# BoothGroup/evcont

Measured on AMD Instinct MI355X. Metric: continuation geometries/sec (energy+force), H30 STO-3G, 20 training states, higher is better.
Workload: dtype f64

## Files before the change

### evcont_amd/csrc/kernels.hpp

```cpp
#pragma once
#include "common.hpp"

namespace evc {

constexpr int kMaxOrbitals = 96;
constexpr int kMaxBatchG = 32;

struct RowProblem {
    const double *A;
    const double *v;
    double *partial;
    int64_t rows, cols, ld, vstride, pstride;
    int nspans, nblocks;
    int64_t span_cols;
    int lds_plan;
};
struct GemvRowsLaunch {
    RowProblem p[2];
    int nblk0;
    int nblk1;
    int tpg[2], trem[2], nrg[2];
};
struct ColProblem {
    const double *A;
    const double *w;
    const double *wt;
    double *out;
    int64_t rows, cols, ld, wstride, ostride;
    double *part;
    int64_t pstride;
};
constexpr int kColSlabs = 64;
struct GemvColsLaunch {
    ColProblem p[2];
    int nblk0;
};
int launch_gemv_rows_mfma(const GemvRowsLaunch &L, int g0, int G, int tiles, hipStream_t st);
int launch_gemv_cols_mfma(GemvColsLaunch L, int g0, int G, hipStream_t st);
void plan_rows(RowProblem &P, bool batched);
bool rows_lds_applicable(const RowProblem &p0, const RowProblem &p1);
void plan_rows_lds(RowProblem &p0, RowProblem &p1);
int rows_max_spans(const RowProblem &P, bool small);
int launch_gemv_rows_lds(const GemvRowsLaunch &L, int g0, int G, hipStream_t st);
int rows_lds_max_g(const RowProblem &p0, const RowProblem &p1);
int cols_lds_mode(const ColProblem &p0, const ColProblem &p1, int G);
int launch_gemv_cols_lds(const GemvColsLaunch &L, int g0, int G, hipStream_t st);
int launch_gemv_cols_lds_slab(const GemvColsLaunch &L, int g0, int G, hipStream_t st);
bool rows_groups_all_mfma(int count);
size_t rows_ws_doubles(int64_t rows, int64_t cols);
int launch_gemv_rows(RowProblem p0, RowProblem p1, int count, hipStream_t st);
int launch_gemv_cols(ColProblem p0, ColProblem p1, int count, hipStream_t st);

int launch_quarter_transform(const double *in, int64_t sin, const double *C, int64_t sC, int c_transposed, int n,
                             double *out, int64_t sout, int count, hipStream_t st);
struct PairTransformArgs {
    const double *in;
    const double *C;
    double *out;
    double *packed;
    double *k3;
    int64_t sin, sC, sout, spacked, sk3, packed_len;
    double diag_mult;
    int ct, n;
    int tiles_per_wg;
    int sym8;
    int lead_sym;
    int in_lower;
    int rs_lower;
    int out_pairs;
    int in_pairs;
    int in_ld, out_ld;
};
__host__ __device__ inline int pair_ld(int n) { return (n * (n + 1) / 2 + 15) & ~15; }
constexpr int kPairTransformMaxN = 32;
constexpr int kPtRawMax = (kPairTransformMaxN * (kPairTransformMaxN + 1) / 2 + 1 + 127) / 128;
constexpr int kPtRowLen = kPtRawMax * 128 + 4;
int launch_pair_transform(const PairTransformArgs &a, int count, hipStream_t st);
bool pair_transform_dma_applicable(const PairTransformArgs &a, int count);
int launch_pair_transform_dma(const PairTransformArgs &a, int count, hipStream_t st);
bool y2_dma_applicable(int n);
int launch_y2_dma(const double *SB, const double *M1, const double *X, int64_t sX, int n, double *partial, int64_t sws,
                  int count, int slabs, int tiles_per_wg, int ppt, hipStream_t st);
int launch_pack(const double *h2, int64_t sh2, int n, double diag_mult, double *out, int64_t sout, int64_t out_len,
                int count, hipStream_t st);
int launch_pack_sym8(const double *h2, int64_t sh2, int n, double diag_mult, double *out, int64_t sout,
                     int64_t out_len, int count, hipStream_t st);
int launch_unpack(const double *packed, int64_t sp, int n, double *out, int64_t sout, int count, hipStream_t st);
int launch_sym_oao_t(const double *G, int64_t sG, int n, double *out, int64_t sout, int count, hipStream_t st);
int launch_unpack_sym(const double *packed, int64_t sp, int n, double *GsT, double *SB, int64_t sws, double *G,
                      int64_t sG, int count, hipStream_t st);
int launch_unpack8(const double *packed, int64_t sp, int n, double *SB, int64_t sws, double *G, int64_t sG, int count,
                   int lead_half, hipStream_t st);
int launch_y2_sb(const double *SB, const double *K3, int n, double *partial, int64_t sws, int count, hipStream_t st);
int launch_y2_fused(const double *SB, const double *M1, const double *X, int64_t sX, int n, double *partial,
                    int64_t sws, int count, hipStream_t st);
int y2_fused_slabs(int n, int count);
bool y2_fused_available(int n);
int y2_slabs(int n);
int y2_slab_capacity(int n);
int launch_y2(const double *GsT, const double *K3, int n, double *partial, int64_t sws, int count, hipStream_t st);
int ip1_chunks(int n);
__host__ __device__ inline int64_t geo_of(int64_t g, int geo_period) { return geo_period > 0 ? g % geo_period : g; }
struct Ip1Args {
    const double *ip1;
    const double *Gao;
    double *t2part;
    const double *dh;
    const double *Pao;
    double *term3;
    const double *y2part;
    double *y2;
    int64_t sip1, sdh, sws;
    int n, natm, nslab, nchunk;
    int presym;
    int fold_cd;
    int ip1_s2kl;
    int geo_period;
    int slots;
};
constexpr int kIp1MaxSlots = 8;
int launch_ip1_dh(const Ip1Args &a, int count, hipStream_t st);

bool pair64_applicable(const PairTransformArgs &a);
int launch_pair_transform64(const PairTransformArgs &a, int count, hipStream_t st);
bool y2_64_applicable(int n);
int y2_64_slabs(int n, int count);
int launch_y2_64(const double *SB, const double *M1, const double *X, int64_t sX, int n, double *partial, int64_t sws,
                 int count, hipStream_t st);

struct LoewdinArgs {
    const double *S, *h;
    double *X, *U, *s, *h1;
    int64_t sS, sh, sws;
    int n;
    int warm;
    int fast;
    double *scratch;
    int64_t sscratch;
    double *flag;
    int part;
};
int launch_loewdin(const LoewdinArgs &a, int count, hipStream_t st);
bool loewdin_split_available(int n);
int launch_loewdin_big(const LoewdinArgs &a, int count, hipStream_t st);
int eigh_fast_enabled();
int subspace_few_enabled();

struct SolveArgs {
    const double *h1part;
    int nsp1;
    double alpha1;
    const double *h2part;
    int nsp2;
    double alpha2;
    const double *S;
    int64_t sS;
    int T, layout, nroots;
    double e_shift;
    const double *e_shift_dev;
    double *evals, *evecs, *Hout;
    double *w2, *w1;
    double *w2t;
    double *w1t;
    int64_t sh1, sh2, sev, svec, sH, sw;
    int64_t w2_offset, w2_count;
    double *vstd;
    int warm;
    int fast;
    double *bcache;
    int few;
    double *scratch;
    int64_t sscratch;
};
constexpr int kSubspaceSmallT = 32;
constexpr int kSubspaceMaxT = 512;
int launch_subspace_loewdin(const SolveArgs &s, const LoewdinArgs &l, int count, hipStream_t st);
int launch_subspace_solve(const SolveArgs &a, int count, hipStream_t st);
size_t subspace_big_scratch_doubles(int T);
int launch_subspace_big(const SolveArgs &a, int count, hipStream_t st);

__host__ __device__ inline bool layout_pairs(int layout) {
    return layout == EVC_LAYOUT_PAIR5 || layout == EVC_LAYOUT_PACK2 || layout == EVC_LAYOUT_SYM8;
}
int launch_pair_weights(const double *c, int T, int layout, double *w1, double *w2, int64_t w2_offset,
                        int64_t w2_count, hipStream_t st);
int launch_pair_weights_geo(const double *c, int64_t sc, int geo_period, int T, int layout, const int32_t *pairs,
                            int npairs, double *w1, double *w2, double *w1t, double *w2t, int64_t sw, int64_t w2_offset,
                            int64_t w2_count, hipStream_t st);
constexpr int kPairWeightsSlots = 256;
struct PairWeightsArgs {
    const double *c;
    double *w1, *w2;
    double *w1t, *w2t;
    int64_t sw, w2_offset, w2_count, sc;
    int T, pairs, slot0, geo_period;
    int16_t k[kPairWeightsSlots], l[kPairWeightsSlots];
};
struct GradPrepArgs {
    int n;
    const double *X;
    const double *hcore;
    const double *D;
    double *Pao;
    double *Y1;
    int64_t sws, sh, sD;
    double scale1;
    int geo_period;
};
int launch_grad_prep(const GradPrepArgs &a, int count, hipStream_t st);
int launch_unpack8_prep(const GradPrepArgs &a, const double *packed, int64_t sp, double *SB, int64_t sws, int count,
                        hipStream_t st);
struct GradFinalArgs {
    int n, natm;
    const double *U, *s;
    const double *Y1;
    const double *y2;
    const double *ipovlp;
    const int64_t *aoslices;
    const double *t2part;
    int nchunk;
    const double *term3;
    const double *gnuc;
    double scale1;
    double *grad;
    int64_t sws, sip, sgn, sgrad;
    int geo_period;
};
int launch_grad_final(const GradFinalArgs &a, int count, hipStream_t st);

}
```

### evcont_amd/csrc/pair_dma.hip

```cpp
#include <stdlib.h>

#include "common.hpp"
#include "kernels.hpp"

namespace evc {

namespace {

typedef double d4 __attribute__((ext_vector_type(4)));
typedef double d2 __attribute__((ext_vector_type(2)));

constexpr int kPdMaxN = 30;
constexpr unsigned kPdRaw = 4;
constexpr unsigned kPdRB = kPdRaw * 1024 + 64;
constexpr unsigned kPdStage = 4 * kPdRB;
constexpr unsigned kPdP = 3872;
constexpr unsigned kPdTab = kPdStage + 16 * kPdP;
constexpr unsigned kPdLds = kPdTab, kPdLds1 = kPdTab + 512 * 4;

__device__ __forceinline__ d4 mfma_f64(double a, double b, d4 c) {
    return __builtin_amdgcn_mfma_f64_16x16x4f64(a, b, c, 0, 0, 0);
}
__device__ __forceinline__ void glds16(unsigned voff, const void *sbase, unsigned lds_addr) {
    asm volatile("s_mov_b32 m0, %2\n\ts_nop 0\n\tglobal_load_lds_dwordx4 %0, %1"
                 :
                 : "v"(voff), "s"(sbase), "s"(lds_addr)
                 : "memory");
}
__device__ __forceinline__ void gstore16(unsigned voff, d2 v, const void *sbase) {
    asm volatile("global_store_dwordx4 %0, %1, %2" : : "v"(voff), "v"(v), "s"(sbase) : "memory");
}
__device__ __forceinline__ unsigned opaque(unsigned x) {
    asm volatile("" : "+v"(x));
    return x;
}
typedef __attribute__((address_space(3))) double lds_f64;
typedef __attribute__((address_space(3))) float lds_f32;
typedef float f2 __attribute__((ext_vector_type(2)));
typedef __attribute__((address_space(3))) f2 lds_f2;
__device__ __forceinline__ double lds_ld(unsigned addr) { return *(lds_f64 *)(uintptr_t)addr; }
__device__ __forceinline__ void lds_st(unsigned addr, double v) { *(lds_f64 *)(uintptr_t)addr = v; }
__device__ __forceinline__ void wait_vm_dyn(int k) {
    if (k <= 0) asm volatile("s_waitcnt vmcnt(0)" ::: "memory");
    else if (k == 1) asm volatile("s_waitcnt vmcnt(1)" ::: "memory");
    else if (k == 2) asm volatile("s_waitcnt vmcnt(2)" ::: "memory");
    else asm volatile("s_waitcnt vmcnt(3)" ::: "memory");
}

#ifdef EVC_PTD_NO_SETPRIO
#define EVC_PTD_PRIO(x_) do { } while (0)
#else
#define EVC_PTD_PRIO(x_) __builtin_amdgcn_s_setprio(x_)
#endif

}

template <int MODE>
__global__ __launch_bounds__(256, 2) void ptd_kernel(PairTransformArgs a) {
    constexpr int KS = 8, NT = 2;
    extern __shared__ __align__(16) char lds[];
    const int n = a.n;
    const int npairs = n * (n + 1) / 2;
    const int in_ld = a.in_ld ? a.in_ld : npairs, out_ld = a.out_ld;
    const int64_t g = blockIdx.y;
    const double *__restrict__ in = a.in + g * a.sin;
    const double *__restrict__ C = a.C + g * a.sC;
    const int ntiles = (npairs + 7) / 8;
    const int t_begin = blockIdx.x * a.tiles_per_wg, t_end = min(ntiles, t_begin + a.tiles_per_wg);
    if (t_begin >= t_end) return;
    const int niter = 2 * (t_end - t_begin);
    const int lane = threadIdx.x & 63;
    const int wave = __builtin_amdgcn_readfirstlane(threadIdx.x >> 6);
    const int l15 = lane & 15, l4 = lane >> 4;

    const int e0 = 8 * t_begin + wave;
    const int dw = (int)(((reinterpret_cast<uintptr_t>(in) >> 3) + (uintptr_t)((int64_t)e0 * in_ld)) & 1);
    const unsigned rowb = (unsigned)wave * kPdRB;
    unsigned fa[NT][KS];
#pragma unroll
    for (int rt = 0; rt < NT; ++rt)
#pragma unroll
        for (int kk = 0; kk < KS; ++kk) {
            const int r = rt * 16 + l15, s = 4 * kk + l4;
            const int hi = s > r ? s : r, lo = s > r ? r : s;
            fa[rt][kk] = (r < n && s < n) ? rowb + 8u * (unsigned)(dw + hi * (hi + 1) / 2 + lo) : rowb + kPdRaw * 1024;
        }
    if (lane < 8) *reinterpret_cast<double *>(lds + rowb + kPdRaw * 1024 + 8 * lane) = 0.0;
    const unsigned wbytes = (unsigned)(((npairs + dw) * 8 + 15) & ~15);
    unsigned vo[kPdRaw];
#pragma unroll
    for (unsigned u = 0; u < kPdRaw; ++u) {
        const unsigned o = 1024u * u + 16u * (unsigned)lane;
        vo[u] = o < wbytes ? o : 0u;
    }
    const int npieces = __builtin_amdgcn_readfirstlane((int)((wbytes + 1023u) >> 10));
    auto dma_row = [&](int e) {
        const int ec = e < npairs ? e : wave;
        const char *src = reinterpret_cast<const char *>(in + (int64_t)ec * in_ld) - 8 * dw;
#pragma unroll
        for (unsigned u = 0; u < kPdRaw; ++u)
            if ((int)u < npieces) glds16(vo[u], src, rowb + 1024u * u);
    };
    dma_row(e0);

    double xf[KS][NT];
#pragma unroll
    for (int kk = 0; kk < KS; ++kk)
#pragma unroll
        for (int t = 0; t < NT; ++t) {
            const int d = 4 * kk + l4, c = t * 16 + l15;
            const bool ok = d < n && c < n;
            const double *src = C + (ok ? (a.ct ? c * n + d : d * n + c) : 0);
            const double v = *src;
            xf[kk][t] = ok ? v : 0.0;
        }

    unsigned sa[2][12];
#pragma unroll
    for (int f = 0; f < 12; ++f) {
        const int tile = f / 4, reg = f % 4;
        const int it = tile == 0 ? 0 : 1, st = tile == 2 ? 1 : 0;
        const int r2 = it * 16 + l4 + 4 * reg, s2 = st * 16 + l15;
        const bool ok = r2 < n && s2 <= r2;
        sa[0][f] = opaque(kPdStage + (unsigned)wave * kPdP + 8u * (unsigned)(ok ? r2 * (r2 + 1) / 2 + s2 : npairs + l15));
        sa[1][f] = opaque(sa[0][f] + 8u * kPdP);
    }
    const int wl = 2 * (threadIdx.x & 3), ur = threadIdx.x >> 2;
    const unsigned wo = opaque(kPdStage + (unsigned)wl * kPdP + 8u * (unsigned)ur);
    const unsigned gvo = (unsigned)((ur * out_ld + wl) * 8);
    char *outg = reinterpret_cast<char *>(MODE == 0 ? a.out + g * a.sout : a.packed + g * a.spacked);
    [[maybe_unused]] unsigned tv[8];
    [[maybe_unused]] double frow[8];
    if constexpr (MODE == 1) {
        for (int u = threadIdx.x; u < 512; u += 256) {
            const int r = tri_row_small(u);
            *(lds_f32 *)(uintptr_t)(kPdTab + 4u * (unsigned)u) = (u == r * (r + 3) / 2) ? 1.0f : 2.0f;
        }
        if (blockIdx.x == 0) {
            double *pk = a.packed + g * a.spacked;
            const int64_t M = (int64_t)npairs * (npairs + 1) / 2;
            for (int64_t m = M + threadIdx.x; m < a.packed_len; m += 256) pk[m] = 0.0;
        }
        __syncthreads();
#pragma unroll
        for (int k = 0; k < 8; ++k) {
            const int u = ur + 64 * k;
            tv[k] = (unsigned)((u * (u + 1) / 2 + wl) * 8);
            frow[k] = (double)*(lds_f32 *)(uintptr_t)(kPdTab + 4u * (unsigned)(u & 511));
        }
    }
    const int wrows = npairs - 16 * wave;
    int vmask = 0;
#pragma unroll
    for (int k = 0; k < 8; ++k) vmask |= (64 * k < wrows) ? 1 << k : 0;
    vmask = __builtin_amdgcn_readfirstlane(vmask);
    int cntA = 0, cntB = 0;
#pragma unroll
    for (int c = 1; c < 4; ++c) {
        cntA += (64 * c < wrows) ? 1 : 0;
        cntB += (64 * (4 + c) < wrows) ? 1 : 0;
    }

    double mf[NT][KS];
    asm volatile("s_waitcnt vmcnt(0)" ::: "memory");
#pragma unroll
    for (int rt = 0; rt < NT; ++rt)
#pragma unroll
        for (int kk = 0; kk < KS; ++kk) mf[rt][kk] = lds_ld(fa[rt][kk]);
    asm volatile("s_waitcnt lgkmcnt(0)" ::: "memory");
    dma_row(e0 + 4);

    d4 nnA[NT][NT], nnB[NT][NT];
#pragma unroll
    for (int it = 0; it < NT; ++it)
#pragma unroll
        for (int st = 0; st < NT; ++st) nnA[it][st] = nnB[it][st] = (d4){0.0, 0.0, 0.0, 0.0};
    const d4 zero = {0.0, 0.0, 0.0, 0.0};

    auto iteration = [&](auto compute_tag, auto ph_tag, const int i, d4 (&nnp)[NT][NT], d4 (&nn)[NT][NT]) {
        constexpr bool COMPUTE = decltype(compute_tag)::value;
        constexpr int PH = decltype(ph_tag)::value;
        constexpr bool ODD = (PH & 1) != 0;
        constexpr unsigned TP = PH >> 1;
        d4 h[NT][NT];
        if constexpr (COMPUTE || !ODD) {
            constexpr unsigned simm = ODD ? 0u : 4u * kPdP, sbuf = ODD ? TP : (TP ^ 1u);
#pragma unroll
            for (int kk = 0; kk < KS; ++kk) {
#pragma unroll
                for (int m = 0; m < NT * NT; ++m) {
                    if constexpr (COMPUTE) {
                        const int rt = m / NT, st = m % NT;
                        EVC_PTD_PRIO(0);
                        h[rt][st] = mfma_f64(mf[rt][kk], xf[kk][st], kk == 0 ? zero : h[rt][st]);
                        EVC_PTD_PRIO(1);
                    }
                    const int f = kk * 2 + m;
                    if (m < 2 && f < 12) {
                        const int tile = f / 4, reg = f % 4;
                        const int it = tile == 0 ? 0 : 1, st2 = tile == 2 ? 1 : 0;
                        lds_st(sa[sbuf][f] + simm, nnp[it][st2][reg]);
                    }
                    __builtin_amdgcn_sched_barrier(0);
                }
            }
        }
        if (!ODD && i >= 2) lds_barrier();
        {
            int act = (ODD ? i >= 3 : i >= 2) ? vmask : 0;
            const int jt = (ODD ? i - 3 : i - 2) >> 1;
            constexpr unsigned bimm = (TP ^ 1u) * 8u * kPdP;
            char *ob = outg + (int64_t)(8 * (t_begin + jt)) * 8;
#ifdef EVC_PTD_K0
            const int K = 0;
#else
            const int K = (MODE == 0 && i >= 3) ? (ODD ? cntA : cntB) : 0;
#endif
            d2 dv[4];
            [[maybe_unused]] int kd = 0;
            [[maybe_unused]] d2 cf = {1.0, 1.0};
            if constexpr (MODE == 1) {
                const int tg = t_begin + (jt < 0 ? 0 : jt);
                kd = tg >> 3;
                act &= ~((1 << kd) - 1);
                ob = outg + (int64_t)(8 * tg) * 8;
                const f2 c2 = *(lds_f2 *)(uintptr_t)(kPdTab + 4u * (unsigned)(8 * tg + wl));
                cf = (d2){(double)c2[0], (double)c2[1]};
            }
            asm volatile("" : "+s"(act));
#pragma unroll
            for (int kk = 0; kk < KS; ++kk) {
                if ((kk & 1) == 0) {
                    const int c = kk / 2, k = (ODD ? 4 : 0) + c;
                    if (act >> k & 1) {
                        dv[c][0] = lds_ld(wo + 512u * k + bimm);
                        dv[c][1] = lds_ld(wo + 512u * k + bimm + kPdP);
                    }
                }
                __builtin_amdgcn_sched_barrier(0);
#pragma unroll
                for (int m = 0; m < 3; ++m) {
                    if constexpr (COMPUTE) {
                        const int it = m == 0 ? 0 : 1, st = m == 2 ? 1 : 0;
                        EVC_PTD_PRIO(0);
                        nn[it][st] = mfma_f64(xf[kk][it], h[kk / 4][st][kk % 4], kk == 0 ? zero : nn[it][st]);
                        EVC_PTD_PRIO(1);
                        if (m == 0) {
                            if (kk == 0) wait_vm_dyn(K);
                            if (kk < 2) {
#pragma unroll
                                for (int k2 = 0; k2 < KS; ++k2)
                                    mf[kk][k2] = lds_ld(fa[kk][k2]);
                            }
                            if (kk == 2) {
                                asm volatile("s_waitcnt lgkmcnt(0)" ::: "memory");
                                dma_row(e0 + 4 * (i + 2));
                            }
                        }
                    }
                    if (m == 2 && (kk & 1) == 1) {
                        const int c = kk / 2, k = (ODD ? 4 : 0) + c;
                        if constexpr (MODE == 0) {
                            if (act >> k & 1) gstore16(gvo, dv[c], ob + (int64_t)(64 * k) * out_ld * 8);
                        } else if (act >> k & 1) {
                            const int u = ur + 64 * k;
                            d2 f = cf * frow[k];
                            if (k != kd) {
                                const d2 v = dv[c] * f;
                                if (u < npairs) gstore16(tv[k], v, ob);
                            } else {
                                const int d = u - (8 * (t_begin + jt) + wl);
                                if (d == 0) f[0] *= a.diag_mult;
                                if (d == 1) f[1] *= a.diag_mult;
                                const d2 v = dv[c] * f;
                                if (u < npairs) {
                                    if (d >= 1) *reinterpret_cast<d2 *>(ob + tv[k]) = v;
                                    else if (d == 0) *reinterpret_cast<double *>(ob + tv[k]) = v[0];
                                }
                            }
                        }
                    }
                    __builtin_amdgcn_sched_barrier(0);
                }
            }
        }
    };
    using T = std::true_type;
    using F = std::false_type;
    using P0 = std::integral_constant<int, 0>;
    using P1 = std::integral_constant<int, 1>;
    using P2 = std::integral_constant<int, 2>;
    using P3 = std::integral_constant<int, 3>;
    int i = 0;
    for (; i + 4 <= niter; i += 4) {
        iteration(T{}, P0{}, i, nnB, nnA);
        iteration(T{}, P1{}, i + 1, nnA, nnB);
        iteration(T{}, P2{}, i + 2, nnB, nnA);
        iteration(T{}, P3{}, i + 3, nnA, nnB);
    }
    if (i < niter) {
        iteration(T{}, P0{}, i, nnB, nnA);
        iteration(T{}, P1{}, i + 1, nnA, nnB);
        iteration(F{}, P2{}, i + 2, nnB, nnA);
        iteration(F{}, P3{}, i + 3, nnA, nnB);
    } else {
        iteration(F{}, P0{}, i, nnB, nnA);
        iteration(F{}, P1{}, i + 1, nnA, nnB);
    }
    asm volatile("s_waitcnt vmcnt(0)" ::: "memory");
}

__global__ __launch_bounds__(256, 2) void y2d_kernel(const double *__restrict__ SB, const double *__restrict__ M1,
                                                     const double *__restrict__ X, int64_t sX, int n,
                                                     double *__restrict__ partial, int64_t sws, int tiles_per_wg, int ppt) {
    constexpr int KS = 8, NT = 2, NPAD = 32;
    extern __shared__ __align__(16) char lds[];
    const int npairs = n * (n + 1) / 2, ld = pair_ld(n);
    const int64_t g = blockIdx.y;
    SB += g * sws;
    M1 += g * sws;
    X += g * sX;
    partial += g * sws;
    const int ntiles = (npairs + ppt - 1) / ppt;
    const int t_begin = blockIdx.x * tiles_per_wg, t_end = min(ntiles, t_begin + tiles_per_wg);
    const int lane = threadIdx.x & 63;
    const int wave = __builtin_amdgcn_readfirstlane(threadIdx.x >> 6);
    const int l15 = lane & 15, l4 = lane >> 4;
    d4 yD[NT][NT], yO[NT][NT];
#pragma unroll
    for (int ti = 0; ti < NT; ++ti)
#pragma unroll
        for (int ta = 0; ta < NT; ++ta) yD[ti][ta] = yO[ti][ta] = (d4){0.0, 0.0, 0.0, 0.0};
    if (t_begin < t_end) {
        const int niter = (ppt / 4) * (t_end - t_begin);
        const unsigned rowM = (unsigned)wave * 2u * kPdRB, rowT = rowM + kPdRB;
        unsigned fa[NT][KS];
#pragma unroll
        for (int rt = 0; rt < NT; ++rt)
#pragma unroll
            for (int kk = 0; kk < KS; ++kk) {
                const int r = rt * 16 + l15, s = 4 * kk + l4;
                const int hi = s > r ? s : r, lo = s > r ? r : s;
                fa[rt][kk] = opaque((r < n && s < n) ? rowM + 8u * (unsigned)(hi * (hi + 1) / 2 + lo) : rowM + kPdRaw * 1024);
            }
        if (lane < 8) {
            *reinterpret_cast<double *>(lds + rowM + kPdRaw * 1024 + 8 * lane) = 0.0;
            *reinterpret_cast<double *>(lds + rowT + kPdRaw * 1024 + 8 * lane) = 0.0;
        }
        const unsigned wbytes = (unsigned)((npairs * 8 + 15) & ~15);
        unsigned vo[kPdRaw];
#pragma unroll
        for (unsigned u = 0; u < kPdRaw; ++u) {
            const unsigned o = 1024u * u + 16u * (unsigned)lane;
            vo[u] = o < wbytes ? o : 0u;
        }
        const int npieces = __builtin_amdgcn_readfirstlane((int)((wbytes + 1023u) >> 10));
        auto dma_row = [&](const double *base, int e, unsigned dst) {
            const char *src = reinterpret_cast<const char *>(base + (int64_t)(e < npairs ? e : wave) * ld);
#pragma unroll
            for (unsigned u = 0; u < kPdRaw; ++u)
                if ((int)u < npieces) glds16(vo[u], src, dst + 1024u * u);
        };
        auto wait_older = [&]() {
            if (npieces >= 4) asm volatile("s_waitcnt vmcnt(4)" ::: "memory");
            else if (npieces == 3) asm volatile("s_waitcnt vmcnt(3)" ::: "memory");
            else if (npieces == 2) asm volatile("s_waitcnt vmcnt(2)" ::: "memory");
            else asm volatile("s_waitcnt vmcnt(1)" ::: "memory");
        };
        const int e0 = ppt * t_begin + wave;
        dma_row(M1, e0, rowM);
        dma_row(SB, e0, rowT);
        double xf[KS][NT];
#pragma unroll
        for (int kk = 0; kk < KS; ++kk)
#pragma unroll
            for (int t = 0; t < NT; ++t) {
                const int d = 4 * kk + l4, c = t * 16 + l15;
                const bool ok = d < n && c < n;
                const double v = X[ok ? d * n + c : 0];
                xf[kk][t] = ok ? v : 0.0;
            }
        double mf[NT][KS], tf[NT][KS];
        asm volatile("s_waitcnt vmcnt(0)" ::: "memory");
#pragma unroll
        for (int rt = 0; rt < NT; ++rt)
#pragma unroll
            for (int kk = 0; kk < KS; ++kk) mf[rt][kk] = lds_ld(fa[rt][kk]);
        asm volatile("s_waitcnt lgkmcnt(0)" ::: "memory");
        dma_row(M1, e0 + 4, rowM);
        int pp = __builtin_amdgcn_readfirstlane(tri_row_small(e0 < npairs ? e0 : 0)), qq = (e0 < npairs ? e0 : 0) - pp * (pp + 1) / 2;
        const d4 zero = {0.0, 0.0, 0.0, 0.0};
        for (int i = 0; i < niter; ++i) {
            const int e = e0 + 4 * i;
            const bool live = e < npairs, diag = qq == pp;
            d4 hT[NT][NT];
#pragma unroll
            for (int kk = 0; kk < KS; ++kk) {
#pragma unroll
                for (int m = 0; m < NT * NT; ++m) {
                    const int it = m / NT, st = m % NT;
                    hT[it][st] = mfma_f64(xf[kk][it], mf[st][kk], kk == 0 ? zero : hT[it][st]);
                    if (m == 0) {
                        if (kk == 0) wait_older();
                        if (kk < 2) {
#pragma unroll
                            for (int k2 = 0; k2 < KS; ++k2) tf[kk][k2] = lds_ld(fa[kk][k2] + kPdRB);
                        }
                        if (kk == 2) {
                            asm volatile("s_waitcnt lgkmcnt(0)" ::: "memory");
                            dma_row(SB, e + 4, rowT);
                        }
                    }
                    __builtin_amdgcn_sched_barrier(0);
                }
            }
            auto yphase = [&](auto live_tag, d4 (&y)[NT][NT]) {
#pragma unroll
                for (int kk = 0; kk < KS; ++kk) {
#pragma unroll
                    for (int m = 0; m < NT * NT; ++m) {
                        const int ti = m / NT, ta = m % NT;
                        if constexpr (decltype(live_tag)::value)
                            y[ti][ta] = mfma_f64(tf[ti][kk], hT[kk / 4][ta][kk % 4], y[ti][ta]);
                        if (m == 0) {
                            if (kk == 0) wait_older();
                            if (kk < 2) {
#pragma unroll
                                for (int k2 = 0; k2 < KS; ++k2) mf[kk][k2] = lds_ld(fa[kk][k2]);
                            }
                            if (kk == 2) {
                                asm volatile("s_waitcnt lgkmcnt(0)" ::: "memory");
                                dma_row(M1, e + 8, rowM);
                            }
                        }
                        __builtin_amdgcn_sched_barrier(0);
                    }
                }
            };
            if (!live) yphase(std::false_type{}, yD);
            else if (diag) yphase(std::true_type{}, yD);
            else yphase(std::true_type{}, yO);
            qq += 4;
            while (qq > pp) {
                qq -= pp + 1;
                ++pp;
            }
        }
        asm volatile("s_waitcnt vmcnt(0)" ::: "memory");
    }
    __syncthreads();
    double *red = reinterpret_cast<double *>(lds);
#pragma unroll
    for (int ti = 0; ti < NT; ++ti)
#pragma unroll
        for (int ta = 0; ta < NT; ++ta)
#pragma unroll
            for (int r = 0; r < 4; ++r)
                red[(wave * NPAD + ti * 16 + l4 + 4 * r) * (NPAD + 1) + ta * 16 + l15] = yD[ti][ta][r] + 2.0 * yO[ti][ta][r];
    __syncthreads();
    double *dst = partial + (int64_t)blockIdx.x * n * n;
    for (int idx = threadIdx.x; idx < n * n; idx += 256) {
        const int i = idx / n, aa = idx % n;
        const int o = i * (NPAD + 1) + aa;
        constexpr int WS = NPAD * (NPAD + 1);
        dst[idx] = (red[o] + red[WS + o]) + (red[2 * WS + o] + red[3 * WS + o]);
    }
}

bool y2_dma_applicable(int n) {
    static const bool on = !(getenv("EVC_PT_DMA") && atoi(getenv("EVC_PT_DMA")) == 0);
    return on && n > 16 && n <= kPdMaxN;
}

int launch_y2_dma(const double *SB, const double *M1, const double *X, int64_t sX, int n, double *partial, int64_t sws,
                  int count, int slabs, int tiles_per_wg, int ppt, hipStream_t st) {
    constexpr unsigned ldsb = 8 * kPdRB > 4 * 32 * 33 * 8 ? 8 * kPdRB : 4 * 32 * 33 * 8;
    hipLaunchKernelGGL(y2d_kernel, dim3((unsigned)slabs, (unsigned)count), dim3(256), ldsb, st, SB, M1, X, sX, n, partial,
                       sws, tiles_per_wg, ppt);
    note_kernel(EVC_PROF_Y2, "y2d_kernel");
    EVC_LAUNCH_CHECK("y2_dma");
    return 0;
}

bool pair_transform_dma_applicable(const PairTransformArgs &a, int count) {
    static const bool on = !(getenv("EVC_PT_DMA") && atoi(getenv("EVC_PT_DMA")) == 0);
    const int npairs = a.n * (a.n + 1) / 2;
    return on && a.n > 16 && a.n <= kPdMaxN && count >= 4 && a.lead_sym && a.in_lower && a.rs_lower && a.in_pairs &&
           !a.k3 && (a.in_ld == 0 || a.in_ld >= npairs) &&
           ((a.out && a.out_pairs && !a.packed && a.out_ld >= 8 * ((npairs + 7) / 8) && a.out_ld % 2 == 0) ||
            (a.packed && a.sym8 && !a.out));
}

int launch_pair_transform_dma(const PairTransformArgs &a_in, int count, hipStream_t st) {
    PairTransformArgs a = a_in;
    const int npairs = a.n * (a.n + 1) / 2, ntiles = (npairs + 7) / 8;
    if (a.tiles_per_wg < 1) a.tiles_per_wg = 4;
    const dim3 grid((unsigned)((ntiles + a.tiles_per_wg - 1) / a.tiles_per_wg), (unsigned)count);
    if (a.packed) {
        static LdsAttr attr1;
        if (int rc = allow_dynamic_lds(ptd_kernel<1>, attr1, 160 * 1024, "pair_transform_dma")) return rc;
        hipLaunchKernelGGL((ptd_kernel<1>), grid, dim3(256), kPdLds1, st, a);
        note_kernel(EVC_PROF_PAIR_TRANSFORM, "ptd_kernel<1>");
    } else {
        static LdsAttr attr;
        if (int rc = allow_dynamic_lds(ptd_kernel<0>, attr, 160 * 1024, "pair_transform_dma")) return rc;
        hipLaunchKernelGGL((ptd_kernel<0>), grid, dim3(256), kPdLds, st, a);
        note_kernel(EVC_PROF_PAIR_TRANSFORM, "ptd_kernel<0>");
    }
    EVC_LAUNCH_CHECK("pair_transform_dma");
    return 0;
}

}
```

### evcont_amd/csrc/pipeline.hip

```cpp
#include <stdlib.h>
#include <string.h>

#include <atomic>
#include <mutex>
#include <unordered_map>

#include "common.hpp"
#include "kernels.hpp"

namespace evc {

static thread_local char g_err[512] = "";
void set_error(const char *fmt, ...) {
    va_list ap;
    va_start(ap, fmt);
    vsnprintf(g_err, sizeof(g_err), fmt, ap);
    va_end(ap);
}

constexpr int kProfStages = 11;
static char g_kernel_ran[kProfStages][96];
void note_kernel(int stage, const char *fmt, ...) {
    if (stage < 0 || stage >= kProfStages) return;
    va_list ap;
// ... 435 lines not shown
        EVC_LAUNCH_CHECK("rows_reduce");
    }
    return 0;
}

static int phase_solve(const evc_trdm_set *t, const Geo &g, const double *h2rows_all, int64_t sh2_all, const Out &out,
                       int nroots, Ws &w, hipStream_t st) {
    SolveArgs a;
    memset(&a, 0, sizeof(a));
    const int64_t sw = w.stride;
    a.h1part = w.h1part;
    a.nsp1 = w.rp1.nspans;
    a.alpha1 = 1.0;
    a.sh1 = sw;
    if (h2rows_all) {
        a.h2part = h2rows_all;
        a.nsp2 = 1;
        a.alpha2 = 1.0;
        a.sh2 = sh2_all;
    } else if (reduce_in_own_launch(w)) {
        a.h2part = w.h2rows;
        a.nsp2 = 1;
        a.alpha2 = 1.0;
        a.sh2 = sw;
    } else {
        a.h2part = w.h2part;
        a.nsp2 = w.rp2.nspans;
        a.alpha2 = is_packed(t->layout) ? 1.0 : 0.5;
        a.sh2 = sw;
    }
    a.S = t->s_train;
    a.T = t->ntrain;
    a.layout = t->layout;
    a.nroots = nroots;
    a.e_shift = g.enuc;
    a.e_shift_dev = g.enuc_dev;
    if (out.energy) {
        a.evals = out.energy;
        a.sev = out.se;
    } else {
        a.evals = w.evals;
        a.sev = sw;
    }
    if (out.coeffs) {
        a.evecs = out.coeffs;
        a.svec = out.sc;
    } else {
        a.evecs = w.evecs;
        a.svec = sw;
    }
    a.Hout = out.hmat;
    a.sH = out.sH;
    a.w2 = w.w2;
    a.w2t = g.count > 1 ? w.w2t : nullptr;
    a.w1t = g.count > 1 ? w.w1t : nullptr;
    a.w1 = w.w1;
    a.sw = sw;
    a.w2_offset = t->row_offset;
    a.w2_count = t->rows2;
    a.vstd = w.vstd;
    a.bcache = w.bcache;
    a.scratch = w.sbig;
    a.sscratch = sw;
    a.warm = w.warm ? 1 : 0;
    const int pr = prof_start(EVC_PROF_SUBSPACE, st);
    const int rc = w.split == 3 ? launch_subspace_loewdin(a, w.la_ride, g.count, st) : launch_subspace_solve(a, g.count, st);
    prof_stop(pr, st);
    return rc;
}

static int gradient_from_rdms(int n, const Geo &g, const double *D, int64_t sD, double *G, int64_t sG,
                              const double *packed, int64_t spacked, int sym8, int ip1_s2kl, double scale1,
                              bool add_gnuc, double *grad, int64_t sgrad, Ws &w, hipStream_t st) {
    const int cnt = g.count;
    const int64_t sw = w.stride;
    int rc;
    double *gao;
    auto rotate_to_ao = [&](const double *src, int64_t ssrc, double *other, double *dst) -> int {
        int r;
        if (use_pair_transform(n)) {
            PairTransformArgs pa;
            memset(&pa, 0, sizeof(pa));
            pa.C = w.X;
            pa.sC = sw;
            pa.ct = 1;
            pa.n = n;
            pa.in = src;
            pa.sin = ssrc;
            pa.out = other;
            pa.sout = sw;
            if ((r = launch_pair_transform(pa, cnt, st))) return r;
            pa.in = other;
            pa.sin = sw;
            pa.out = dst;
            return launch_pair_transform(pa, cnt, st);
        }
        if ((r = launch_quarter_transform(src, ssrc, w.X, sw, 1, n, dst, sw, cnt, st))) return r;
        if ((r = launch_quarter_transform(dst, sw, w.X, sw, 1, n, other, sw, cnt, st))) return r;
        if ((r = launch_quarter_transform(other, sw, w.X, sw, 1, n, dst, sw, cnt, st))) return r;
        if ((r = launch_quarter_transform(dst, sw, w.X, sw, 1, n, other, sw, cnt, st))) return r;
        return 1 << 30;
    };
    GradPrepArgs p;
    p.n = n;
    p.X = w.X;
    p.hcore = g.hcore;
    p.D = D;
    p.Pao = w.Pao;
    p.Y1 = w.Y1;
    p.sws = sw;
    p.sh = g.sh;
    p.sD = sD;
    p.scale1 = scale1;
    p.geo_period = g.geo_period;
    const bool prep_with_unpack = packed && sym8 && !G && use_pair_transform(n);
    if (!prep_with_unpack && (rc = launch_grad_prep(p, cnt, st))) return rc;
    const bool p64 = packed && use_pair64(sym8 ? EVC_LAYOUT_SYM8 : 0, n, ip1_s2kl != 0);
    const bool pairs_route = use_pair_transform(n) || p64;
    const bool fused_y2 = packed && pairs_route && use_fused_y2(sym8 != 0, n);
    int y2_slabs_used = y2_slabs(n);
    auto ip1_stage = [&](const double *gao_, int c0, int cc) -> int {
        const int64_t o = (int64_t)c0 * sw;
        EVC_REQUIRE(g.geo_period == 0 || (c0 == 0 && cc == cnt), "gradient: geometry-mapped slots in chunks");
        Ip1Args ia;
        ia.ip1 = g.eri_ip1 + (int64_t)c0 * g.sip1;
        ia.Gao = gao_ + o;
        ia.presym = packed ? 1 : 0;
        ia.fold_cd = (packed && sym8 && pairs_route) ? 1 : 0;
        ia.ip1_s2kl = ip1_s2kl;
        ia.t2part = w.t2part + o;
        ia.dh = g.dhcore ? g.dhcore + (int64_t)c0 * g.sdh : nullptr;
        ia.Pao = w.Pao + o;
        ia.term3 = w.term3 + o;
        ia.y2part = w.y2part + o;
        ia.y2 = w.y2 + o;
        ia.sip1 = g.sip1;
        ia.sdh = g.sdh;
        ia.sws = sw;
        ia.n = n;
        ia.natm = g.natm;
        ia.nslab = y2_slabs_used;
        ia.nchunk = ip1_chunks(n);
        ia.geo_period = g.geo_period;
        ia.slots = g.geo_period > 0 ? cnt / g.geo_period : 1;
        return launch_ip1_dh(ia, cc, st);
    };
    bool ip1_done = false;
    if (packed) {
        if (pairs_route) {
            const int chunk = cnt;
            for (int c0 = 0; c0 < cnt; c0 += chunk) {
                const int cc = cnt - c0 < chunk ? cnt - c0 : chunk;
                const int64_t o = (int64_t)c0 * sw;
                int pr = prof_start(EVC_PROF_UNPACK, st);
                if (sym8) {
                    if (prep_with_unpack && c0 == 0 && cc == cnt) {
                        if ((rc = launch_unpack8_prep(p, packed, spacked, w.B1, sw, cnt, st))) return rc;
                    } else {
                        if (prep_with_unpack && c0 == 0 && (rc = launch_grad_prep(p, cnt, st))) return rc;
                        if ((rc = launch_unpack8(packed + (int64_t)c0 * spacked, spacked, n, (G && p64 ? w.B2 : w.B1) + o, sw,
                                                 G ? G + (int64_t)c0 * sG : nullptr, sG, cc, G ? 1 : 2, st)))
                            return rc;
                    }
                    if (G && p64 &&
                        (rc = launch_unpack8(packed + (int64_t)c0 * spacked, spacked, n, w.B1 + o, sw, nullptr, 0, cc, 2, st)))
                        return rc;
                    prof_stop(pr, st);
                    pr = prof_start(EVC_PROF_Y2, st);
                    if (fused_y2) {
                        const double *sbp = w.B1 + o;
                        if (G && !p64) {
                            if ((rc = launch_unpack8(packed + (int64_t)c0 * spacked, spacked, n, w.B2 + o, sw, nullptr, 0,
                                                     cc, 2, st)))
                                return rc;
                            sbp = w.B2 + o;
                        }
                        if ((rc = launch_y2_fused(sbp, w.K3 + o, w.X + o, sw, n, w.y2part + o, sw, cc, st))) return rc;
                        y2_slabs_used = y2_fused_slabs(n, cc);
                    } else {
                        set_error("gradient: the symmetric pipeline needs the fused Y2 contraction (n <= 32)");
                        return -1;
                    }
                } else {
                    if ((rc = launch_unpack_sym(packed + (int64_t)c0 * spacked, spacked, n, w.B2 + o, w.B1 + o, sw,
                                                G ? G + (int64_t)c0 * sG : nullptr, sG, cc, st)))
                        return rc;
                    prof_stop(pr, st);
                    pr = prof_start(EVC_PROF_Y2, st);
                    if ((rc = launch_y2(w.B2 + o, w.K3 + o, n, w.y2part + o, sw, cc, st))) return rc;
                }
                prof_stop(pr, st);
                PairTransformArgs pa;
                memset(&pa, 0, sizeof(pa));
                pa.C = w.X + o;
                pa.sC = sw;
                pa.ct = 1;
                pa.n = n;
                pa.in = w.B1 + o;
                pa.sin = sw;
                pa.out = w.B2 + o;
                pa.sout = sw;
                pa.lead_sym = pa.in_lower = pa.rs_lower = sym8;
                pa.in_pairs = (sym8 && (!G || p64)) ? 1 : 0;
                pa.out_pairs = sym8;
                pa.in_ld = pa.out_ld = pair_ld(n);
                pr = prof_start(EVC_PROF_PAIR_TRANSFORM, st);
                if ((rc = launch_pair_transform(pa, cc, st))) return rc;
                prof_stop(pr, st);
                pa.in = w.B2 + o;
                pa.out = w.B1 + o;
                pa.in_pairs = pa.out_pairs;
                pa.out_pairs = ip1_s2kl ? 1 : 0;
                pr = prof_start(EVC_PROF_PAIR_TRANSFORM, st);
                if ((rc = launch_pair_transform(pa, cc, st))) return rc;
                prof_stop(pr, st);
                pr = prof_start(EVC_PROF_IP1, st);
                if ((rc = ip1_stage(w.B1, c0, cc))) return rc;
                prof_stop(pr, st);
            }
            ip1_done = true;
        } else {
            if (sym8) {
                if ((rc = launch_unpack8(packed, spacked, n, w.B1, sw, G, sG, cnt, 0, st))) return rc;
                if ((rc = launch_y2_sb(w.B1, w.K3, n, w.y2part, sw, cnt, st))) return rc;
            } else {
                if ((rc = launch_unpack_sym(packed, spacked, n, w.B2, w.B1, sw, G, sG, cnt, st))) return rc;
                if ((rc = launch_y2(w.B2, w.K3, n, w.y2part, sw, cnt, st))) return rc;
            }
            if ((rc = launch_quarter_transform(w.B1, sw, w.X, sw, 1, n, w.B2, sw, cnt, st))) return rc;
            if ((rc = launch_quarter_transform(w.B2, sw, w.X, sw, 1, n, w.B1, sw, cnt, st))) return rc;
            if ((rc = launch_quarter_transform(w.B1, sw, w.X, sw, 1, n, w.B2, sw, cnt, st))) return rc;
            if ((rc = launch_quarter_transform(w.B2, sw, w.X, sw, 1, n, w.B1, sw, cnt, st))) return rc;
        }
        gao = w.B1;
    } else {
        if ((rc = launch_sym_oao_t(G, sG, n, w.B2, sw, cnt, st))) return rc;
        if ((rc = launch_y2(w.B2, w.K3, n, w.y2part, sw, cnt, st))) return rc;
        rc = rotate_to_ao(G, sG, w.B1, w.B2);
        if (rc == (1 << 30)) gao = w.B1;
        else if (rc) return rc;
        else gao = w.B2;
    }
    if (!ip1_done && (rc = ip1_stage(gao, 0, cnt))) return rc;
    if ((rc = side_join(w.base, st))) return rc;
    GradFinalArgs f;
    f.n = n;
    f.natm = g.natm;
    f.U = w.U;
    f.s = w.s;
    f.Y1 = w.Y1;
    f.y2 = w.y2;
    f.ipovlp = g.ipovlp;
    f.aoslices = g.aoslices;
    f.t2part = w.t2part;
    f.nchunk = ip1_chunks(n);
    f.term3 = w.term3;
    f.gnuc = add_gnuc ? g.gnuc : nullptr;
    f.scale1 = scale1;
    f.grad = grad;
    f.sws = sw;
    f.sip = g.sip;
    f.sgn = g.sgn;
    f.sgrad = sgrad;
    f.geo_period = g.geo_period;
    return launch_grad_final(f, cnt, st);
}

static int phase_gradient(const evc_trdm_set *t, const Geo &g_in, const Out &out, int flags, Ws &w, hipStream_t st) {
    const int n = t->n, cnt = g_in.count;
    Geo g = g_in;
    const int s2kl = (flags & EVC_FLAG_IP1_S2KL) ? 1 : 0;
    if (s2kl) {
        EVC_REQUIRE(is_sym8(t->layout) && (use_pair_transform(n) || use_pair64(t->layout, n, true)),
                    "EVC_FLAG_IP1_S2KL needs the compressed layout (EVC_LAYOUT_SYM8) and N <= 64");
        if (cnt > 1 && g.sip1) g.sip1 = (int64_t)3 * n * n * (n * (n + 1) / 2);
    }
    const int64_t sw = w.stride;
    int rc;
    double *D = out.d_pred ? out.d_pred : w.Dpred;
    const int64_t sD = out.d_pred ? out.sd : sw;
    double *G = out.g_pred ? out.g_pred : w.G;
    const int64_t sG = out.g_pred ? out.sG : sw;
    ColProblem c2{}, c1{};
    c2.A = t->two_rdm;
    c2.w = w.w2;
    c2.wt = cnt > 1 ? w.w2t : nullptr;
    c2.wstride = sw;
    c2.rows = t->rows2;
    c2.cols = t->cols2;
    c2.ld = t->ld2;
    if (is_packed(t->layout)) {
        c2.out = w.vec2;
        c2.ostride = sw;
    } else {
        c2.out = G;
        c2.ostride = sG;
    }
    c1.A = t->one_rdm;
    c1.w = w.w1;
    c1.wt = cnt > 1 ? w.w1t : nullptr;
    c1.wstride = sw;
    c1.rows = (int64_t)t->ntrain * t->ntrain;
    c1.cols = (int64_t)n * n;
    c1.ld = t->ld1;
    c1.out = D;
    c1.ostride = sD;
    c1.part = (int64_t)t->ntrain * t->ntrain >= 1024 ? w.d1part : nullptr;
    c1.pstride = sw;
    const int pr = prof_start(EVC_PROF_COLS, st);
    if ((rc = launch_gemv_cols(c2, c1, cnt, st))) return rc;
    prof_stop(pr, st);
    const bool partial = (flags & EVC_FLAG_PARTIAL_RANK) != 0;
    if (is_packed(t->layout))
        return gradient_from_rdms(n, g, D, sD, out.g_pred, out.sG, w.vec2, sw, is_sym8(t->layout) ? 1 : 0, s2kl,
                                  partial ? 0.0 : 1.0, !partial, out.grad, out.sg, w, st);
    return gradient_from_rdms(n, g, D, sD, G, sG, nullptr, 0, 0, 0, partial ? 0.0 : 1.0, !partial, out.grad, out.sg,
                              w, st);
}

static Geo geo_single(const evc_geometry *g) {
    Geo o;
    memset(&o, 0, sizeof(o));
    if (!g) return o;
    o.natm = g->natm;
    o.count = 1;
    o.S = g->S;
    o.hcore = g->hcore;
    o.eri = g->eri;
    o.ipovlp = g->ipovlp;
    o.dhcore = g->dhcore;
    o.eri_ip1 = g->eri_ip1;
    o.gnuc = g->gnuc;
    o.aoslices = g->aoslices;
    o.enuc = g->enuc;
    return o;
}

static Geo geo_batch(const evc_trdm_set *t, const evc_geometry_batch *gb) {
    Geo g;
    memset(&g, 0, sizeof(g));
    if (!t || !gb) return g;
    const int64_t n2 = (int64_t)t->n * t->n, n4 = n2 * n2, A3 = (int64_t)gb->natm * 3;
    g.natm = gb->natm;
    g.count = gb->count;
    g.batch = 1;
    g.S = gb->S;
    g.sS = n2;
    g.hcore = gb->hcore;
    g.sh = n2;
    g.eri = gb->eri;
    g.seri = n4;
    g.ipovlp = gb->ipovlp;
    g.sip = 3 * n2;
    g.dhcore = gb->dhcore;
    g.sdh = A3 * n2;
    g.eri_ip1 = gb->eri_ip1;
    g.sip1 = 3 * n4;
    g.gnuc = gb->gnuc;
    g.sgn = A3;
    g.aoslices = gb->aoslices;
    g.enuc_dev = gb->enuc;
// ... 627 lines not shown
```

Before: 82870.

## Fuse Y2 contraction into the first dense pair-transform step kernel

Adds a Y2 phase to the DMA pair-transform kernel body so that one launch streams the pair rows, performs the first dense transform step, and accumulates the Y2 partial contraction from the same LDS-resident tiles plus a DMA'd M1 row. The pipeline then skips the separate fused-Y2 launch and the first pair-transform launch when applicable. The aim is to remove one kernel launch and a second full read of the unpacked two-electron tensor. In exchange the kernel uses more LDS and runs at one block per CU, which may reduce occupancy.

```diff
diff --git a/evcont_amd/csrc/kernels.hpp b/evcont_amd/csrc/kernels.hpp
--- a/evcont_amd/csrc/kernels.hpp
+++ b/evcont_amd/csrc/kernels.hpp
@@ -81,6 +81,10 @@
 bool y2_dma_applicable(int n);
 int launch_y2_dma(const double *SB, const double *M1, const double *X, int64_t sX, int n, double *partial, int64_t sws,
                   int count, int slabs, int tiles_per_wg, int ppt, hipStream_t st);
+bool y2_pairstep_applicable(const PairTransformArgs &a, const double *M1, int64_t sws, int count);
+int y2_pairstep_slabs(int n, int count);
+int launch_y2_pairstep(const PairTransformArgs &a, const double *M1, double *partial, int64_t sws, int count,
+                       hipStream_t st);
 int launch_pack(const double *h2, int64_t sh2, int n, double diag_mult, double *out, int64_t sout, int64_t out_len,
                 int count, hipStream_t st);
 int launch_pack_sym8(const double *h2, int64_t sh2, int n, double diag_mult, double *out, int64_t sout,
diff --git a/evcont_amd/csrc/pair_dma.hip b/evcont_amd/csrc/pair_dma.hip
--- a/evcont_amd/csrc/pair_dma.hip
+++ b/evcont_amd/csrc/pair_dma.hip
@@ -17,6 +17,10 @@
 constexpr unsigned kPdP = 3872;
 constexpr unsigned kPdTab = kPdStage + 16 * kPdP;
 constexpr unsigned kPdLds = kPdTab, kPdLds1 = kPdTab + 512 * 4;
+constexpr unsigned kPdStageY = 8 * kPdRB;
+constexpr unsigned kPdSqP = 34, kPdSqB = 32 * kPdSqP * 8;
+constexpr unsigned kPdSq = kPdStageY + 16 * kPdP;
+constexpr unsigned kPdLdsY = kPdSq + 4 * kPdSqB;
 
 __device__ __forceinline__ d4 mfma_f64(double a, double b, d4 c) {
     return __builtin_amdgcn_mfma_f64_16x16x4f64(a, b, c, 0, 0, 0);
@@ -46,6 +50,14 @@
     else if (k == 2) asm volatile("s_waitcnt vmcnt(2)" ::: "memory");
     else asm volatile("s_waitcnt vmcnt(3)" ::: "memory");
 }
+__device__ __forceinline__ void wait_vm_dyn8(int k) {
+    if (k <= 3) wait_vm_dyn(k);
+    else if (k == 4) asm volatile("s_waitcnt vmcnt(4)" ::: "memory");
+    else if (k == 5) asm volatile("s_waitcnt vmcnt(5)" ::: "memory");
+    else if (k == 6) asm volatile("s_waitcnt vmcnt(6)" ::: "memory");
+    else if (k == 7) asm volatile("s_waitcnt vmcnt(7)" ::: "memory");
+    else asm volatile("s_waitcnt vmcnt(8)" ::: "memory");
+}
 
 #ifdef EVC_PTD_NO_SETPRIO
 #define EVC_PTD_PRIO(x_) do { } while (0)
@@ -55,9 +67,18 @@
 
 }
 
-template <int MODE>
-__global__ __launch_bounds__(256, 2) void ptd_kernel(PairTransformArgs a) {
+struct Y2dArgs {
+    const double *SB, *M1, *X;
+    double *partial;
+    int64_t sX, sws;
+    int n, tiles_per_wg, ppt;
+};
+
+template <int MODE, bool Y2>
+__device__ __forceinline__ void ptd_body(const PairTransformArgs &a, const Y2dArgs &y) {
     constexpr int KS = 8, NT = 2;
+    constexpr unsigned kPdStage = Y2 ? kPdStageY : evc::kPdStage;
+    static_assert(!Y2 || MODE == 0, "the Y2 phase belongs to the dense step");
     extern __shared__ __align__(16) char lds[];
     const int n = a.n;
     const int npairs = n * (n + 1) / 2;
@@ -67,7 +88,13 @@
     const double *__restrict__ C = a.C + g * a.sC;
     const int ntiles = (npairs + 7) / 8;
     const int t_begin = blockIdx.x * a.tiles_per_wg, t_end = min(ntiles, t_begin + a.tiles_per_wg);
-    if (t_begin >= t_end) return;
+    if (t_begin >= t_end) {
+        if constexpr (Y2) {
+            double *dst = y.partial + g * y.sws + (int64_t)blockIdx.x * n * n;
+            for (int idx = threadIdx.x; idx < n * n; idx += 256) dst[idx] = 0.0;
+        }
+        return;
+    }
     const int niter = 2 * (t_end - t_begin);
     const int lane = threadIdx.x & 63;
     const int wave = __builtin_amdgcn_readfirstlane(threadIdx.x >> 6);
@@ -102,6 +129,19 @@
             if ((int)u < npieces) glds16(vo[u], src, rowb + 1024u * u);
     };
     dma_row(e0);
+    [[maybe_unused]] const double *__restrict__ M1 = Y2 ? y.M1 + g * y.sws : nullptr;
+    constexpr unsigned kRowM = 4 * kPdRB;
+    [[maybe_unused]] auto dma_mrow = [&](int e) {
+        const int ec = e < npairs ? e : wave;
+        const char *src = reinterpret_cast<const char *>(M1 + (int64_t)ec * in_ld);
+#pragma unroll
+        for (unsigned u = 0; u < kPdRaw; ++u)
+            if ((int)u < npieces) glds16(vo[u], src, rowb + kRowM + 1024u * u);
+    };
+    if constexpr (Y2) {
+        if (lane < 8) *reinterpret_cast<double *>(lds + rowb + kRowM + kPdRaw * 1024 + 8 * lane) = 0.0;
+        dma_mrow(e0);
+    }
 
     double xf[KS][NT];
 #pragma unroll
@@ -159,6 +199,25 @@
     for (int c = 1; c < 4; ++c) {
         cntA += (64 * c < wrows) ? 1 : 0;
         cntB += (64 * (4 + c) < wrows) ? 1 : 0;
+    }
+    [[maybe_unused]] unsigned sqw[4] = {0, 0, 0, 0}, sqr[2] = {0, 0};
+    if constexpr (Y2) {
+        const unsigned sq = kPdSq + (unsigned)wave * kPdSqB;
+#pragma unroll
+        for (int b = 0; b < 4; ++b) sqw[b] = opaque(sq + 8u * (unsigned)((l4 + 8 * b) * (int)kPdSqP + l15));
+#pragma unroll
+        for (int b = 0; b < 2; ++b) sqr[b] = opaque(sq + 8u * (unsigned)((l15 + 16 * b) * (int)kPdSqP + l4));
+    }
+    [[maybe_unused]] double mb[NT][KS], ha[NT][KS];
+    [[maybe_unused]] d4 yy[NT][NT];
+    [[maybe_unused]] int pp = 0, qq = 0;
+    if constexpr (Y2) {
+        pp = __builtin_amdgcn_readfirstlane(tri_row_small(e0 < npairs ? e0 : 0));
+        qq = (e0 < npairs ? e0 : 0) - pp * (pp + 1) / 2;
+#pragma unroll
+        for (int ti = 0; ti < NT; ++ti)
+#pragma unroll
+            for (int ta = 0; ta < NT; ++ta) yy[ti][ta] = (d4){0.0, 0.0, 0.0, 0.0};
     }
 
     double mf[NT][KS];
@@ -246,7 +305,10 @@
                         nn[it][st] = mfma_f64(xf[kk][it], h[kk / 4][st][kk % 4], kk == 0 ? zero : nn[it][st]);
                         EVC_PTD_PRIO(1);
                         if (m == 0) {
-                            if (kk == 0) wait_vm_dyn(K);
+                            if (kk == 0) {
+                                if constexpr (Y2) wait_vm_dyn8(i == 0 ? 0 : K + npieces);
+                                else wait_vm_dyn(K);
+                            }
                             if (kk < 2) {
 #pragma unroll
                                 for (int k2 = 0; k2 < KS; ++k2)
@@ -256,6 +318,25 @@
                                 asm volatile("s_waitcnt lgkmcnt(0)" ::: "memory");
                                 dma_row(e0 + 4 * (i + 2));
                             }
+                        }
+                    }
+                    if constexpr (COMPUTE && Y2) {
+                        if (m == 1) {
+                            if (kk < 4) {
+#pragma unroll
+                                for (int reg = 0; reg < 4; ++reg)
+                                    lds_st(sqw[2 * (kk / 2) + reg / 2] + 8u * (4u * (reg % 2) * kPdSqP + 16u * (kk % 2)), h[kk / 2][kk % 2][reg]);
+                            } else {
+                                const int rt = kk & 1, k0 = kk < 6 ? 0 : 4;
+#pragma unroll
+                                for (int k2 = k0; k2 < k0 + 4; ++k2)
+                                    ha[rt][k2] = lds_ld(sqr[rt] + 8u * 4u * k2);
+                            }
+                        }
+                        if (m == 0 && kk == 7) {
+                            wait_vm_dyn8(npieces + __builtin_popcount((unsigned)(act >> (ODD ? 4 : 0)) & 7u));
+                            mb[0][0] = lds_ld(fa[0][0] + kRowM);
+                            mb[1][0] = lds_ld(fa[1][0] + kRowM);
                         }
                     }
                     if (m == 2 && (kk & 1) == 1) {
@@ -284,6 +365,51 @@
                 }
             }
         }
+        if constexpr (COMPUTE && Y2) {
+            auto yphase = [&](auto live_tag, auto diag_tag) {
+                constexpr bool LIVE = decltype(live_tag)::value, DIAG = decltype(diag_tag)::value;
+                if constexpr (DIAG) {
+                    mb[0][0] *= 0.5;
+                    mb[1][0] *= 0.5;
+                }
+#pragma unroll
+                for (int kk = 0; kk < KS; ++kk)
+#pragma unroll
+                    for (int m = 0; m < NT * NT; ++m) {
+                        const int ti = m / NT, ta = m % NT;
+                        if constexpr (LIVE) {
+                            EVC_PTD_PRIO(0);
+                            yy[ti][ta] = mfma_f64(ha[ti][kk], mb[ta][kk], yy[ti][ta]);
+                            EVC_PTD_PRIO(1);
+                            if (m == 0 && kk < KS - 1) {
+                                mb[0][kk + 1] = lds_ld(fa[0][kk + 1] + kRowM);
+                                mb[1][kk + 1] = lds_ld(fa[1][kk + 1] + kRowM);
+                            }
+                            if constexpr (DIAG) {
+                                if (m == 3 && kk < KS - 1) {
+                                    mb[0][kk + 1] *= 0.5;
+                                    mb[1][kk + 1] *= 0.5;
+                                }
+                            }
+                        }
+                        if (m == 1 && kk == KS - 1) {
+                            asm volatile("s_waitcnt lgkmcnt(0)" ::: "memory");
+                            dma_mrow(e0 + 4 * (i + 1));
+                        }
+                        __builtin_amdgcn_sched_barrier(0);
+                    }
+            };
+            using Tt = std::true_type;
+            using Ff = std::false_type;
+            if (e0 + 4 * i >= npairs) yphase(Ff{}, Ff{});
+            else if (qq == pp) yphase(Tt{}, Tt{});
+            else yphase(Tt{}, Ff{});
+            qq += 4;
+            while (qq > pp) {
+                qq -= pp + 1;
+                ++pp;
+            }
+        }
     };
     using T = std::true_type;
     using F = std::false_type;
@@ -308,11 +434,43 @@
         iteration(F{}, P1{}, i + 1, nnA, nnB);
     }
     asm volatile("s_waitcnt vmcnt(0)" ::: "memory");
-}
-
-__global__ __launch_bounds__(256, 2) void y2d_kernel(const double *__restrict__ SB, const double *__restrict__ M1,
-                                                     const double *__restrict__ X, int64_t sX, int n,
-                                                     double *__restrict__ partial, int64_t sws, int tiles_per_wg, int ppt) {
+    if constexpr (Y2) {
+        constexpr int NPAD = 32;
+        __syncthreads();
+        double *red = reinterpret_cast<double *>(lds);
+#pragma unroll
+        for (int ti = 0; ti < NT; ++ti)
+#pragma unroll
+            for (int ta = 0; ta < NT; ++ta)
+#pragma unroll
+                for (int r = 0; r < 4; ++r)
+                    red[(wave * NPAD + ti * 16 + l4 + 4 * r) * (NPAD + 1) + ta * 16 + l15] = 2.0 * yy[ti][ta][r];
+        __syncthreads();
+        double *dst = y.partial + g * y.sws + (int64_t)blockIdx.x * n * n;
+        for (int idx = threadIdx.x; idx < n * n; idx += 256) {
+            const int ii = idx / n, aa = idx % n;
+            const int o = ii * (NPAD + 1) + aa;
+            constexpr int WS = NPAD * (NPAD + 1);
+            dst[idx] = (red[o] + red[WS + o]) + (red[2 * WS + o] + red[3 * WS + o]);
+        }
+    }
+}
+
+template <int MODE>
+__global__ __launch_bounds__(256, 2) void ptd_kernel(PairTransformArgs a) {
+    ptd_body<MODE, false>(a, Y2dArgs{});
+}
+
+template <int PS>
+__global__ __launch_bounds__(256, PS ? 1 : 2) void y2d_kernel(Y2dArgs ya, PairTransformArgs pa) {
+    if constexpr (PS) {
+        ptd_body<0, true>(pa, ya);
+        return;
+    }
+    const double *__restrict__ SB = ya.SB, *__restrict__ M1 = ya.M1, *__restrict__ X = ya.X;
+    double *__restrict__ partial = ya.partial;
+    const int64_t sX = ya.sX, sws = ya.sws;
+    const int n = ya.n, tiles_per_wg = ya.tiles_per_wg, ppt = ya.ppt;
     constexpr int KS = 8, NT = 2, NPAD = 32;
     extern __shared__ __align__(16) char lds[];
     const int npairs = n * (n + 1) / 2, ld = pair_ld(n);
@@ -475,10 +633,43 @@
 int launch_y2_dma(const double *SB, const double *M1, const double *X, int64_t sX, int n, double *partial, int64_t sws,
                   int count, int slabs, int tiles_per_wg, int ppt, hipStream_t st) {
     constexpr unsigned ldsb = 8 * kPdRB > 4 * 32 * 33 * 8 ? 8 * kPdRB : 4 * 32 * 33 * 8;
-    hipLaunchKernelGGL(y2d_kernel, dim3((unsigned)slabs, (unsigned)count), dim3(256), ldsb, st, SB, M1, X, sX, n, partial,
-                       sws, tiles_per_wg, ppt);
+    Y2dArgs ya{SB, M1, X, partial, sX, sws, n, tiles_per_wg, ppt};
+    hipLaunchKernelGGL((y2d_kernel<0>), dim3((unsigned)slabs, (unsigned)count), dim3(256), ldsb, st, ya, PairTransformArgs{});
     note_kernel(EVC_PROF_Y2, "y2d_kernel");
     EVC_LAUNCH_CHECK("y2_dma");
+    return 0;
+}
+
+static bool y2_pairstep_on() {
+    static const bool on = !(getenv("EVC_Y2_PAIRSTEP") && atoi(getenv("EVC_Y2_PAIRSTEP")) == 0);
+    return on;
+}
+static int y2_pairstep_tiles(int count) { return count >= 32 ? 8 : count >= 8 ? 4 : 2; }
+
+int y2_pairstep_slabs(int n, int count) {
+    const int ntiles = (n * (n + 1) / 2 + 7) / 8, t = y2_pairstep_tiles(count);
+    return (ntiles + t - 1) / t;
+}
+
+bool y2_pairstep_applicable(const PairTransformArgs &a, const double *M1, int64_t sws, int count) {
+    const int npairs = a.n * (a.n + 1) / 2;
+    const bool aligned = ((reinterpret_cast<uintptr_t>(a.in) | reinterpret_cast<uintptr_t>(M1)) & 15) == 0 &&
+                         a.in_ld >= npairs && a.in_ld % 2 == 0 && a.sin % 2 == 0 && sws % 2 == 0;
+    return y2_pairstep_on() && y2_dma_applicable(a.n) && pair_transform_dma_applicable(a, count) && a.out && a.ct == 1 &&
+           aligned && a.in != a.out && y2_pairstep_slabs(a.n, count) <= y2_slab_capacity(a.n);
+}
+
+int launch_y2_pairstep(const PairTransformArgs &a_in, const double *M1, double *partial, int64_t sws, int count,
+                       hipStream_t st) {
+    PairTransformArgs a = a_in;
+    a.tiles_per_wg = y2_pairstep_tiles(count);
+    Y2dArgs ya{a.in, M1, a.C, partial, a.sC, sws, a.n, a.tiles_per_wg, 8};
+    static LdsAttr attr;
+    if (int rc = allow_dynamic_lds(y2d_kernel<1>, attr, 160 * 1024, "y2_pairstep")) return rc;
+    hipLaunchKernelGGL((y2d_kernel<1>), dim3((unsigned)y2_pairstep_slabs(a.n, count), (unsigned)count), dim3(256), kPdLdsY,
+                       st, ya, a);
+    note_kernel(EVC_PROF_Y2, "y2d_kernel<1> pairstep");
+    EVC_LAUNCH_CHECK("y2_pairstep");
     return 0;
 }
 
diff --git a/evcont_amd/csrc/pipeline.hip b/evcont_amd/csrc/pipeline.hip
--- a/evcont_amd/csrc/pipeline.hip
+++ b/evcont_amd/csrc/pipeline.hip
@@ -611,6 +611,20 @@
             for (int c0 = 0; c0 < cnt; c0 += chunk) {
                 const int cc = cnt - c0 < chunk ? cnt - c0 : chunk;
                 const int64_t o = (int64_t)c0 * sw;
+                PairTransformArgs first;
+                memset(&first, 0, sizeof(first));
+                first.C = w.X + o;
+                first.sC = sw;
+                first.ct = 1;
+                first.n = n;
+                first.in = w.B1 + o;
+                first.sin = sw;
+                first.out = w.B2 + o;
+                first.sout = sw;
+                first.lead_sym = first.in_lower = first.rs_lower = sym8;
+                first.out_pairs = sym8;
+                first.in_ld = first.out_ld = pair_ld(n);
+                bool pairstep = false;
                 int pr = prof_start(EVC_PROF_UNPACK, st);
                 if (sym8) {
                     if (prep_with_unpack && c0 == 0 && cc == cnt) {
@@ -627,15 +641,22 @@
                     prof_stop(pr, st);
                     pr = prof_start(EVC_PROF_Y2, st);
                     if (fused_y2) {
+                        first.in_pairs = sym8;
+                        pairstep = y2_pairstep_applicable(first, w.K3 + o, sw, cc);
                         const double *sbp = w.B1 + o;
                         if (G && !p64) {
-                            if ((rc = launch_unpack8(packed + (int64_t)c0 * spacked, spacked, n, w.B2 + o, sw, nullptr, 0,
-                                                     cc, 2, st)))
+                            double *dense = (pairstep ? w.B1 : w.B2) + o;
+                            if ((rc = launch_unpack8(packed + (int64_t)c0 * spacked, spacked, n, dense, sw, nullptr, 0, cc, 2, st)))
                                 return rc;
-                            sbp = w.B2 + o;
+                            sbp = dense;
                         }
-                        if ((rc = launch_y2_fused(sbp, w.K3 + o, w.X + o, sw, n, w.y2part + o, sw, cc, st))) return rc;
-                        y2_slabs_used = y2_fused_slabs(n, cc);
+                        if (pairstep) {
+                            if ((rc = launch_y2_pairstep(first, w.K3 + o, w.y2part + o, sw, cc, st))) return rc;
+                            y2_slabs_used = y2_pairstep_slabs(n, cc);
+                        } else {
+                            if ((rc = launch_y2_fused(sbp, w.K3 + o, w.X + o, sw, n, w.y2part + o, sw, cc, st))) return rc;
+                            y2_slabs_used = y2_fused_slabs(n, cc);
+                        }
                     } else {
                         set_error("gradient: the symmetric pipeline needs the fused Y2 contraction (n <= 32)");
                         return -1;
@@ -649,23 +670,13 @@
                     if ((rc = launch_y2(w.B2 + o, w.K3 + o, n, w.y2part + o, sw, cc, st))) return rc;
                 }
                 prof_stop(pr, st);
-                PairTransformArgs pa;
-                memset(&pa, 0, sizeof(pa));
-                pa.C = w.X + o;
-                pa.sC = sw;
-                pa.ct = 1;
-                pa.n = n;
-                pa.in = w.B1 + o;
-                pa.sin = sw;
-                pa.out = w.B2 + o;
-                pa.sout = sw;
-                pa.lead_sym = pa.in_lower = pa.rs_lower = sym8;
+                PairTransformArgs pa = first;
                 pa.in_pairs = (sym8 && (!G || p64)) ? 1 : 0;
-                pa.out_pairs = sym8;
-                pa.in_ld = pa.out_ld = pair_ld(n);
-                pr = prof_start(EVC_PROF_PAIR_TRANSFORM, st);
-                if ((rc = launch_pair_transform(pa, cc, st))) return rc;
-                prof_stop(pr, st);
+                if (!pairstep) {
+                    pr = prof_start(EVC_PROF_PAIR_TRANSFORM, st);
+                    if ((rc = launch_pair_transform(pa, cc, st))) return rc;
+                    prof_stop(pr, st);
+                }
                 pa.in = w.B2 + o;
                 pa.out = w.B1 + o;
                 pa.in_pairs = pa.out_pairs;
```

Result: faster. 84740 (median of 6 runs) (+2.3%).
